# neu-vi/Superpoints_Registration

Hardware: AMD Instinct MI355X
Metric: point-cloud pairs/sec (16 384 pts/cloud) (higher is better)
Workload: dtype f32 (matrix products: range-scaled split-f16x2 MFMA, f32 accumulate; attention weights below 2^-5 of their row sum carried in one f16 plane); 1 GPU; synthetic 16384-pt pairs, full KPConv backbone + superpoint attn + Sinkhorn-SVD pose (3dmatch config, BASELINE configs[1]); streams_per_gpu=1, points_per_cloud=16384, generator=box, point_order=reference, upsample_indices=True, cross_step_overlap=True, streams_inside_a_forward=3: main path, pyramid searches, ResNet shortcut branches

## Files before the change

### superpoints_registration_amd/csrc/linear.hip

```cpp
#include <atomic>

#include "attn_planes.h"
#include "lds_dma.h"
#include "spr_common.h"
#include "split_mma.h"

namespace spr {
namespace {

constexpr int BK = 32;
static_assert(BK == kPlaneK, "the split kernels stage split_mma.h's slabs");
constexpr int LDSK = BK + 1;

template <int ACT, bool RES>
__device__ __forceinline__ float store_tile(const f32x16& acc, int row0, int col, int M, int N,
                                            float bv, const float* __restrict__ residual,
                                            float* __restrict__ out, int lh, float unscale = 1.0f,
                                            const float* __restrict__ epi = nullptr) {
  if (col >= N) return 0.f;
  float vmax = 0.f;
  float res[16];
  if (RES) {
#pragma unroll
    for (int r = 0; r < 16; ++r) {
// ... 174 lines not shown

  f32x4 ra[BM * BK / 4 / NT], rb[BN * BK / 4 / NT];
  auto load_slab = [&](int k0) {
    slab_load<BM, NT>(ra, X, M, K, tid, m0, k0);
    slab_load<BN, NT>(rb, Wt, N, K, tid, n0, k0);
  };
  auto store_slab = [&]() {
    wait_vm<0>();
    __builtin_amdgcn_sched_barrier(0);
    slab_store<BM, NT>(ra, sa, Ah, Al, tid);
    slab_store<BN, NT>(rb, sb, Bh, Bl, tid);
  };

  load_slab(0);
  for (int k0 = 0; k0 < K; k0 += BK) {
    store_slab();
    __syncthreads();
    if (k0 + BK < K) load_slab(k0 + BK);
    __builtin_amdgcn_sched_barrier(0);
#pragma unroll
    for (int s = 0; s < BK / 16; ++s) {
      const int ko = 16 * s + 8 * lh;
      f16x8 ah[TM], al[TM], bh[TN], bl[TN];
#pragma unroll
      for (int i = 0; i < TM; ++i) frag_ld40(Ah, Al, (wm * TM + i) * 32 + l31, ko, ah[i], al[i]);
#pragma unroll
      for (int j = 0; j < TN; ++j) frag_ld40(Bh, Bl, (wn * TN + j) * 32 + l31, ko, bh[j], bl[j]);
#pragma unroll
      for (int i = 0; i < TM; ++i)
#pragma unroll
        for (int j = 0; j < TN; ++j) {
          if (PLANES) acc[i][j] = mma3_32<true>(bh[j], bl[j], ah[i], al[i], acc[i][j]);
          else acc[i][j] = mma3_32(ah[i], al[i], bh[j], bl[j], acc[i][j]);
        }
    }
    __builtin_amdgcn_sched_barrier(0);
    __syncthreads();
  }
  wait_vm<0>();
  if (PLANES) {
#pragma unroll
    for (int i = 0; i < TM; ++i) {
      const int tok = m0 + (wm * TM + i) * 32 + l31;
      if (tok >= M) continue;
      const int which = (f0 + n0) >> 8;
      const float pmul = pl.scales[which];
      int vcol = 0;
      if (which == 2) {
        const int sg = find_segment(pl.cu, pl.nseg, tok);
        vcol = attn_vperm(attn_vstart_of(pl.cu[sg], sg) + tok - pl.cu[sg]);
      }
#pragma unroll
      for (int j = 0; j < TN; ++j) {
        const int fl = n0 + (wn * TN + j) * 32;
        const int fg = (f0 + fl) & 255;
        if (which == 2) {
#pragma unroll
          for (int r = 0; r < 16; r += 2) {
            const int d = acc_row32(r, lh);
            const float a = acc[i][j][r] * unscale + bias[fl + d];
            const float b = acc[i][j][r + 1] * unscale + bias[fl + d + 1];
            unsigned int hu, lu;
            split_pk_s(a, b, pmul, hu, lu);
            const f16x2 hh = __builtin_bit_cast(f16x2, hu), ll = __builtin_bit_cast(f16x2, lu);
            const size_t o = attn_v_off(fg + d, (size_t)vcol, 256);
            pl.vth[o] = hh[0];
            pl.vth[o + 16] = hh[1];
            pl.vtl[o] = ll[0];
            pl.vtl[o + 16] = ll[1];
          }
        } else {
          _Float16* ph = which == 0 ? pl.qh : pl.kh;
          _Float16* pw = which == 0 ? pl.ql : pl.kl;
          const size_t row = ((size_t)(fg >> 5) * pl.t_total + tok) * 32;
#pragma unroll
          for (int g = 0; g < 4; ++g) {
            const int d0 = 8 * g + 4 * lh;
            f32x4 v;
#pragma unroll
            for (int e = 0; e < 4; ++e) v[e] = acc[i][j][4 * g + e] * unscale + bias[fl + d0 + e];
            split_store4(v, pmul, ph + row + d0, pw + row + d0);
          }
        }
      }
    }
    return;
  }
  float omax = 0.f;
#pragma unroll
  for (int j = 0; j < TN; ++j) {
    const int col = n0 + (wn * TN + j) * 32 + l31;
    const float bv = (ACT < kEpiScale && bias && col < N) ? bias[col] : 0.f;
#pragma unroll
    for (int i = 0; i < TM; ++i)
      omax = fmaxf(omax, store_tile<ACT, RES>(acc[i][j], m0 + (wm * TM + i) * 32, col, M, N, bv, residual, out, lh,
                                              unscale, ACT >= kEpiScale ? bias : nullptr));
  }
  if (out_parts != nullptr) {
    float* shf = reinterpret_cast<float*>(gemm_smem);
    omax = wave_max(omax);
    __syncthreads();
    if (lane == 0) shf[wave] = omax;
    __syncthreads();
    if (tid == 0) {
      float t = shf[0];
      for (int w_ = 1; w_ < WM * WN; ++w_) t = fmaxf(t, shf[w_]);
      out_parts[blockIdx.x] = t;
    }
  }
}

template <int ACT>
__global__ __launch_bounds__(512) void k_gemm_nt_h3p(
    const float* __restrict__ X, int M, const float* __restrict__ Wt, int N,
    const float* __restrict__ bias, float* __restrict__ out,
    const float* __restrict__ a_parts, int n_aparts, const float* __restrict__ w_parts, int n_wparts,
    float* __restrict__ out_parts, int ntiles) {
  constexpr int K = 256, NSLAB = K / BK;
  constexpr int BM = 128, BN = 256, WN = 4, NT = 512, TM = 2, TN = 2;
  constexpr int QPS = 16 / NSLAB;
  extern __shared__ __align__(16) unsigned char gemm_smem[];
  _Float16* Ah = reinterpret_cast<_Float16*>(gemm_smem);
  _Float16* Al = Ah + BM * kPlaneStride;
  _Float16* Bh = Al + BM * kPlaneStride;
  _Float16* Bl = Bh + BN * kPlaneStride;
  const int tid = threadIdx.x, wave = tid >> 6, lane = tid & 63;
  const int wm = wave / WN, wn = wave % WN;
  const int l31 = lane & 31, lh = lane >> 5;
  const int gx = (N + BN - 1) / BN;

  float sa, sb, unscale;
  {
    float* shf = reinterpret_cast<float*>(gemm_smem);
    const int ka = pow2_exp_for(block_absmax(a_parts, shf, n_aparts));
    const int kb = pow2_exp_for(block_absmax(w_parts, shf, n_wparts));
    __syncthreads();
    sa = pow2f(ka);
    sb = pow2f(kb);
    unscale = pow2f(-ka - kb);
  }

  f32x16 acc[TM][TN], prev[TM][TN];
  f32x4 ra[BM * BK / 4 / NT], rb[BN * BK / 4 / NT];
  auto load_slab = [&](int m0, int n0, int k0) {
    slab_load<BM, NT>(ra, X, M, K, tid, m0, k0);
    slab_load<BN, NT>(rb, Wt, N, K, tid, n0, k0);
  };
  auto store_slab = [&]() {
    slab_store<BM, NT>(ra, sa, Ah, Al, tid);
    slab_store<BN, NT>(rb, sb, Bh, Bl, tid);
  };

  bool have_prev = false;
  int pm0 = 0, pn0 = 0, ptile = 0;
  float pbias[TN] = {0.f, 0.f};
  float pmax = 0.f;
  auto emit = [&](auto qtag) {
    constexpr int Q = decltype(qtag)::value;
    constexpr int b = Q >> 2, g = Q & 3, bi = b >> 1, bj = b & 1;
    const int row0 = pm0 + (wm * TM + bi) * 32 + 8 * g + 4 * lh;
    const int col = pn0 + (wn * TN + bj) * 32 + l31;
    if (col < N) {
      float* p = out + (size_t)row0 * N + col;
#pragma unroll
      for (int e = 0; e < 4; ++e) {
        float y = prev[bi][bj][4 * g + e] * unscale + pbias[bj];
        if (ACT == SPR_ACT_RELU) y = fmaxf(y, 0.f);
        if (ACT == SPR_ACT_SIGMOID) y = 1.f / (1.f + expf(-y));
        if (row0 + e < M) {
          asm volatile("global_store_dword %0, %1, off" ::"v"(p + (size_t)e * N), "v"(y) : "memory");
          pmax = fmaxf(pmax, fabsf(y));
        }
      }
    }
  };
  auto publish_prev_max = [&]() {
    if (out_parts == nullptr) return;
    float* shf = reinterpret_cast<float*>(gemm_smem);
    const float t_ = wave_max(pmax);
    __syncthreads();
    if (lane == 0) shf[wave] = t_;
    __syncthreads();
    if (tid == 0) {
      float m_ = shf[0];
      for (int w_ = 1; w_ < 8; ++w_) m_ = fmaxf(m_, shf[w_]);
      out_parts[ptile] = m_;
    }
    __syncthreads();
    pmax = 0.f;
  };

  int t = blockIdx.x;
  if (t < ntiles) {
    const int lid = xcd_swizzle(t, ntiles);
    load_slab((lid / gx) * BM, (lid % gx) * BN, 0);
  }
  bool young = false;
  for (; t < ntiles; t += gridDim.x) {
    const int lid = xcd_swizzle(t, ntiles);
    const int m0 = (lid / gx) * BM, n0 = (lid % gx) * BN;
    const int tn = t + gridDim.x;
    int nm0 = 0, nn0 = 0;
    if (tn < ntiles) {
      const int nl = xcd_swizzle(tn, ntiles);
      nm0 = (nl / gx) * BM;
      nn0 = (nl % gx) * BN;
    }
#pragma unroll
    for (int i = 0; i < TM; ++i)
#pragma unroll
      for (int j = 0; j < TN; ++j)
#pragma unroll
        for (int r = 0; r < 16; ++r) acc[i][j][r] = 0.f;
    auto slab = [&](auto stag) {
      constexpr int S = decltype(stag)::value;
      if (young) wait_vm<8>();
      else wait_vm<0>();
      __builtin_amdgcn_sched_barrier(0);
      store_slab();
      __syncthreads();
      if (S + 1 < NSLAB) load_slab(m0, n0, (S + 1) * BK);
      else if (tn < ntiles) load_slab(nm0, nn0, 0);
      __builtin_amdgcn_sched_barrier(0);
#pragma unroll
      for (int ks = 0; ks < BK / 16; ++ks) {
        const int ko = 16 * ks + 8 * lh;
        f16x8 ah[TM], al[TM], bh[TN], bl[TN];
#pragma unroll
        for (int i = 0; i < TM; ++i) frag_ld40(Ah, Al, (wm * TM + i) * 32 + l31, ko, ah[i], al[i]);
#pragma unroll
        for (int j = 0; j < TN; ++j) frag_ld40(Bh, Bl, (wn * TN + j) * 32 + l31, ko, bh[j], bl[j]);
#pragma unroll
        for (int i = 0; i < TM; ++i)
#pragma unroll
          for (int j = 0; j < TN; ++j) acc[i][j] = mma3_32(ah[i], al[i], bh[j], bl[j], acc[i][j]);
      }
      __builtin_amdgcn_sched_barrier(0);
      young = false;
      if (have_prev) {
        emit(std::integral_constant<int, QPS * S>{});
        emit(std::integral_constant<int, QPS * S + 1>{});
        young = true;
      }
      __builtin_amdgcn_sched_barrier(0);
      __syncthreads();
    };
    slab(std::integral_constant<int, 0>{});
    slab(std::integral_constant<int, 1>{});
    slab(std::integral_constant<int, 2>{});
    slab(std::integral_constant<int, 3>{});
    slab(std::integral_constant<int, 4>{});
    slab(std::integral_constant<int, 5>{});
    slab(std::integral_constant<int, 6>{});
    slab(std::integral_constant<int, 7>{});
    if (have_prev) publish_prev_max();
#pragma unroll
    for (int i = 0; i < TM; ++i)
#pragma unroll
      for (int j = 0; j < TN; ++j) prev[i][j] = acc[i][j];
    pm0 = m0;
    pn0 = n0;
    ptile = t;
#pragma unroll
    for (int j = 0; j < TN; ++j) {
      const int col = n0 + (wn * TN + j) * 32 + l31;
      pbias[j] = (bias && col < N) ? bias[col] : 0.f;
    }
    have_prev = true;
  }
  if (have_prev) {
    emit(std::integral_constant<int, 0>{});  emit(std::integral_constant<int, 1>{});
    emit(std::integral_constant<int, 2>{});  emit(std::integral_constant<int, 3>{});
    emit(std::integral_constant<int, 4>{});  emit(std::integral_constant<int, 5>{});
    emit(std::integral_constant<int, 6>{});  emit(std::integral_constant<int, 7>{});
    emit(std::integral_constant<int, 8>{});  emit(std::integral_constant<int, 9>{});
    emit(std::integral_constant<int, 10>{}); emit(std::integral_constant<int, 11>{});
    emit(std::integral_constant<int, 12>{}); emit(std::integral_constant<int, 13>{});
    emit(std::integral_constant<int, 14>{}); emit(std::integral_constant<int, 15>{});
    publish_prev_max();
  }
}

static std::atomic<int> g_gemm_mode{1};

__global__ void k_gemv_rows(const float* __restrict__ X, int M, int K, const float* __restrict__ Wt,
                            int N, const float* __restrict__ bias,
                            const float* __restrict__ residual, int act, float* __restrict__ out) {
  const long wid = ((long)blockIdx.x * blockDim.x + threadIdx.x) >> 6;
  const int lane = threadIdx.x & 63;
  if (wid >= (long)M * N) return;
  const int row = (int)(wid / N), n = (int)(wid % N);
  float s = 0.f;
  for (int k = lane; k < K; k += 64) s += X[(size_t)row * K + k] * Wt[(size_t)n * K + k];
  s = wave_sum(s);
  if (lane == 0) {
    float v = s + (bias ? bias[n] : 0.f);
    if (residual) v += residual[(size_t)row * N + n];
    if (act == SPR_ACT_RELU) v = fmaxf(v, 0.f);
    if (act == SPR_ACT_SIGMOID) v = 1.f / (1.f + expf(-v));
    out[(size_t)row * N + n] = v;
  }
}

constexpr int kLnRangeSlots = kRangeSlots;
template <int MAXV>
__global__ void k_layernorm(const float* __restrict__ x, int m, int c,
                            const float* __restrict__ gamma, const float* __restrict__ beta,
                            float eps, const float* __restrict__ pos, float* __restrict__ out_norm,
                            float* __restrict__ out_pos, float* __restrict__ range_norm,
                            float* __restrict__ range_pos) {
  __shared__ float shr[8];
  const int row = (blockIdx.x * blockDim.x + threadIdx.x) >> 6;
  const int lane = threadIdx.x & 63;
  float mxn = 0.f, mxp = 0.f;
  if (row < m) {
  const int nv = c >> 6;
  float v[MAXV];
  float s = 0.f;
#pragma unroll
  for (int i = 0; i < MAXV; ++i) {
    v[i] = (i < nv) ? x[(size_t)row * c + i * 64 + lane] : 0.f;
    s += v[i];
  }
  const float mean0 = wave_sum(s) / (float)c;
  float sd = 0.f;
#pragma unroll
  for (int i = 0; i < MAXV; ++i) sd += (i < nv) ? v[i] - mean0 : 0.f;
  const float mean = mean0 + wave_sum(sd) / (float)c;
  float ss = 0.f;
#pragma unroll
  for (int i = 0; i < MAXV; ++i) {
    const float d = (i < nv) ? v[i] - mean : 0.f;
    ss += d * d;
  }
  const float rstd = 1.0f / sqrtf(wave_sum(ss) / (float)c + eps);
#pragma unroll
  for (int i = 0; i < MAXV; ++i) {
    if (i < nv) {
      const int ch = i * 64 + lane;
      const float y = (v[i] - mean) * rstd * gamma[ch] + beta[ch];
      mxn = fmaxf(mxn, fabsf(y));
      if (out_norm) out_norm[(size_t)row * c + ch] = y;
      if (out_pos) {
        const float yp = y + pos[(size_t)row * c + ch];
        mxp = fmaxf(mxp, fabsf(yp));
        out_pos[(size_t)row * c + ch] = yp;
      }
    }
  }
  }
  if (range_norm || range_pos) {
    mxn = wave_max(mxn);
    mxp = wave_max(mxp);
    if (lane == 0) {
      shr[threadIdx.x >> 6] = mxn;
      shr[4 + (threadIdx.x >> 6)] = mxp;
    }
    __syncthreads();
    if (threadIdx.x == 0) {
      const int slot = blockIdx.x & (kLnRangeSlots - 1);
      if (range_norm)
        atomicMax(reinterpret_cast<unsigned int*>(range_norm) + slot,
                  __float_as_uint(fmaxf(fmaxf(shr[0], shr[1]), fmaxf(shr[2], shr[3]))));
      if (range_pos)
        atomicMax(reinterpret_cast<unsigned int*>(range_pos) + slot,
                  __float_as_uint(fmaxf(fmaxf(shr[4], shr[5]), fmaxf(shr[6], shr[7]))));
    }
  }
}

constexpr int kLnRows = 4;
__global__ __launch_bounds__(256) void k_layernorm256(const float* __restrict__ x, int m,
                                                      const float* __restrict__ gamma,
                                                      const float* __restrict__ beta, float eps,
                                                      const float* __restrict__ pos, float* __restrict__ out_norm,
                                                      float* __restrict__ out_pos, float* __restrict__ range_norm,
                                                      float* __restrict__ range_pos) {
  __shared__ float shr[8];
  const int row0 = ((blockIdx.x * blockDim.x + threadIdx.x) >> 6) * kLnRows;
  const int lane = threadIdx.x & 63;
  float mxn = 0.f, mxp = 0.f;
  float4 v[kLnRows], pv[kLnRows];
#pragma unroll
  for (int r = 0; r < kLnRows; ++r) {
    if (row0 + r < m) {
      const size_t o = (size_t)(row0 + r) * 256 + 4 * lane;
      v[r] = *reinterpret_cast<const float4*>(x + o);
      if (out_pos) pv[r] = *reinterpret_cast<const float4*>(pos + o);
    }
  }
  const float4 g = *reinterpret_cast<const float4*>(gamma + 4 * lane);
  const float4 b = *reinterpret_cast<const float4*>(beta + 4 * lane);
#pragma unroll
  for (int r = 0; r < kLnRows; ++r) {
    if (row0 + r >= m) continue;
    const size_t o = (size_t)(row0 + r) * 256 + 4 * lane;
    const float mean0 = wave_sum((v[r].x + v[r].y) + (v[r].z + v[r].w)) / 256.0f;
    const float mean = mean0 + wave_sum(((v[r].x - mean0) + (v[r].y - mean0)) + ((v[r].z - mean0) + (v[r].w - mean0))) / 256.0f;
    const float dx = v[r].x - mean, dy = v[r].y - mean, dz = v[r].z - mean, dw = v[r].w - mean;
    const float rstd = 1.0f / sqrtf(wave_sum((dx * dx + dy * dy) + (dz * dz + dw * dw)) / 256.0f + eps);
    float4 y;
    y.x = dx * rstd * g.x + b.x;
    y.y = dy * rstd * g.y + b.y;
    y.z = dz * rstd * g.z + b.z;
    y.w = dw * rstd * g.w + b.w;
    mxn = fmaxf(mxn, fmaxf(fmaxf(fabsf(y.x), fabsf(y.y)), fmaxf(fabsf(y.z), fabsf(y.w))));
    if (out_norm) *reinterpret_cast<float4*>(out_norm + o) = y;
    if (out_pos) {
      float4 yp;
      yp.x = y.x + pv[r].x;
      yp.y = y.y + pv[r].y;
      yp.z = y.z + pv[r].z;
      yp.w = y.w + pv[r].w;
      mxp = fmaxf(mxp, fmaxf(fmaxf(fabsf(yp.x), fabsf(yp.y)), fmaxf(fabsf(yp.z), fabsf(yp.w))));
      *reinterpret_cast<float4*>(out_pos + o) = yp;
    }
  }
  if (range_norm || range_pos) {
    mxn = wave_max(mxn);
    mxp = wave_max(mxp);
    if (lane == 0) {
      shr[threadIdx.x >> 6] = mxn;
      shr[4 + (threadIdx.x >> 6)] = mxp;
    }
    __syncthreads();
    if (threadIdx.x == 0) {
      const int slot = blockIdx.x & (kLnRangeSlots - 1);
      if (range_norm)
        atomicMax(reinterpret_cast<unsigned int*>(range_norm) + slot,
                  __float_as_uint(fmaxf(fmaxf(shr[0], shr[1]), fmaxf(shr[2], shr[3]))));
      if (range_pos)
        atomicMax(reinterpret_cast<unsigned int*>(range_pos) + slot,
                  __float_as_uint(fmaxf(fmaxf(shr[4], shr[5]), fmaxf(shr[6], shr[7]))));
    }
  }
}

__global__ void k_posemb(const float* __restrict__ xyz, int n, int d_model, int npf, float scale,
                         float temperature, float* __restrict__ out) {
  const long gid = (long)blockIdx.x * blockDim.x + threadIdx.x;
  if (gid >= (long)n * d_model) return;
  const int row = (int)(gid / d_model), ch = (int)(gid % d_model);
  float v = 0.f;
  if (ch < 3 * npf) {
    const int axis = ch / npf, i = ch % npf;
    const float e = (float)(2 * (i / 2)) / (float)npf;
    const float dim_t = powf(temperature, e);
    const float a = (xyz[3 * (size_t)row + axis] * scale) / dim_t;
    v = (i & 1) ? cosf(a) : sinf(a);
  }
  out[gid] = v;
}

}
}

using namespace spr;

namespace {
template <int ACT, bool RES>
int launch_gemm(const float* x, int m, int k, const float* w, int n, const float* bias,
                const float* residual, float* out, const float* a_parts, int n_aparts, const float* w_parts,
                int n_wparts, float* out_parts, int out_cap, int* out_n, hipStream_t stream) {
  if (out_n) *out_n = 0;
  if (spr::g_gemm_mode.load(std::memory_order_relaxed) == 1) {
    SPR_REQUIRE(a_parts != nullptr && w_parts != nullptr, "linear: split-fp16 mode needs the absmax partials");
    auto lds = [](int bm, int bn) { return (size_t)(bm + bn) * spr::kPlaneStride * 2 * sizeof(_Float16); };
    if (!RES && ACT <= SPR_ACT_SIGMOID && n >= 256 && k == 256 && m >= 1024 && m < 32768) {
      auto kern = spr::k_gemm_nt_h3p<ACT>;
      if (int rc = ensure_dyn_lds((const void*)kern, (int)lds(128, 256))) return rc;
      const int ntiles = cdiv(n, 256) * cdiv(m, 128);
      int grid = device_cu_count();
      grid = grid < ntiles ? grid : ntiles;
      if (grid >= 8) grid &= ~7;
      float* op = (out_parts && ntiles <= out_cap) ? out_parts : nullptr;
      if (op && out_n) *out_n = ntiles;
      hipLaunchKernelGGL(kern, dim3(grid), dim3(512), lds(128, 256), stream, x, m, w, n, bias, out,
                         a_parts, n_aparts, w_parts, n_wparts, op, ntiles);
    } else if (n >= 256 && m >= 256 && cdiv(n, 256) * cdiv(m, 256) >= 128) {
      auto kern = spr::k_gemm_nt_h3<256, 256, 4, 2, ACT, RES>;
      if (int rc = ensure_dyn_lds((const void*)kern, (int)lds(256, 256))) return rc;
      const int grid = cdiv(n, 256) * cdiv(m, 256);
      float* op = (out_parts && grid <= out_cap) ? out_parts : nullptr;
      if (op && out_n) *out_n = grid;
      hipLaunchKernelGGL(kern, dim3(grid), dim3(512), lds(256, 256), stream, x, m, k,
                         w, n, bias, residual, out, spr::AttnPlanes(), 0, a_parts, n_aparts, w_parts, op, (const spr::GemmGroup*)nullptr, n_wparts);
    } else if (n > 32) {
      const int grid = cdiv(n, 64) * cdiv(m, 128);
      float* op = (out_parts && grid <= out_cap) ? out_parts : nullptr;
      if (op && out_n) *out_n = grid;
      hipLaunchKernelGGL((spr::k_gemm_nt_h3<128, 64, 4, 1, ACT, RES>), dim3(grid),
                         dim3(256), lds(128, 64), stream, x, m, k, w, n, bias, residual, out, spr::AttnPlanes(), 0,
                         a_parts, n_aparts, w_parts, op, (const spr::GemmGroup*)nullptr, n_wparts);
    } else {
      hipLaunchKernelGGL((spr::k_gemm_nt_h3<128, 32, 4, 1, ACT, RES>), dim3(cdiv(n, 32) * cdiv(m, 128)),
                         dim3(256), lds(128, 32), stream, x, m, k, w, n, bias, residual, out, spr::AttnPlanes(), 0,
                         a_parts, n_aparts, w_parts, (float*)nullptr, (const spr::GemmGroup*)nullptr, n_wparts);
    }
  } else if (n % 64 == 0) {
    hipLaunchKernelGGL((spr::k_gemm_nt<2, 2, ACT, RES>), dim3((n / 64) * cdiv(m, 64)), dim3(256), 0, stream,
                       x, m, k, w, n, bias, residual, out);
  } else {
    hipLaunchKernelGGL((spr::k_gemm_nt<4, 1, ACT, RES>), dim3(cdiv(n, 32) * cdiv(m, 128)), dim3(256), 0,
                       stream, x, m, k, w, n, bias, residual, out);
  }
  SPR_LAUNCH_CHECK();
  return 0;
}
}

int spr::gemm_mode() { return spr::g_gemm_mode.load(std::memory_order_relaxed); }

int spr::launch_inproj_planes(const float* x, int m, int k, const float* w, int n, const float* bias, int f0,
                              const AttnPlanes& planes, const float* a_parts, int n_aparts, const float* w_parts,
                              hipStream_t stream) {
  SPR_REQUIRE(n % 256 == 0 && f0 % 256 == 0 && k % BK == 0 && m >= 1 && bias != nullptr,
              "in-projection planes: bad shape (m=%d k=%d n=%d)", m, k, n);
  SPR_REQUIRE(a_parts && w_parts && planes.scales, "in-projection planes: missing scale inputs");
  auto kern = spr::k_gemm_nt_h3<256, 256, 4, 2, SPR_ACT_NONE, false, true>;
  const size_t lds = (size_t)(256 + 256) * spr::kPlaneStride * 2 * sizeof(_Float16);
  if (int rc = ensure_dyn_lds((const void*)kern, (int)lds)) return rc;
  hipLaunchKernelGGL(kern, dim3(cdiv(n, 256) * cdiv(m, 256)), dim3(512), lds, stream, x, m, k, w, n, bias,
                     (const float*)nullptr, (float*)nullptr, planes, f0, a_parts, n_aparts, w_parts, (float*)nullptr,
                     (const spr::GemmGroup*)nullptr, kAmaxParts);
  SPR_LAUNCH_CHECK();
  return 0;
}

int spr::launch_linear_ranged(const float* x, int m, int k, const float* w, int n, const float* bias,
                              float* out, const float* a_parts, const float* w_parts, hipStream_t stream) {
  return launch_gemm<SPR_ACT_NONE, false>(x, m, k, w, n, bias, nullptr, out, a_parts, kAmaxParts, w_parts, kAmaxParts,
                                          nullptr, 0, nullptr, stream);
}

void spr::gemm_group_tile(int max_n, int* bm, int* bn) {
  if (max_n >= 256) { *bm = 256; *bn = 256; }
  else if (max_n > 32) { *bm = 128; *bn = 64; }
  else { *bm = 128; *bn = 32; }
}

namespace {
template <int ACT>
int launch_grouped_act(const float* a, int k, const float* b, float* c, const spr::GemmGroup* groups_dev,
                       int total_tiles, int max_n, const float* a_parts, const float* w_parts, const float* epi,
                       hipStream_t stream) {
  auto lds = [](int bm, int bn) { return (size_t)(bm + bn) * spr::kPlaneStride * 2 * sizeof(_Float16); };
  int bm, bn;
  spr::gemm_group_tile(max_n, &bm, &bn);
  if (bn == 256) {
    auto kern = spr::k_gemm_nt_h3<256, 256, 4, 2, ACT, false>;
    if (int rc = ensure_dyn_lds((const void*)kern, (int)lds(256, 256))) return rc;
    hipLaunchKernelGGL(kern, dim3(total_tiles), dim3(512), lds(256, 256), stream, a, 0, k, b, 0, epi,
                       (const float*)nullptr, c, spr::AttnPlanes(), 0, a_parts, kAmaxParts, w_parts,
                       (float*)nullptr, groups_dev, kAmaxParts);
  } else if (bn == 64) {
    hipLaunchKernelGGL((spr::k_gemm_nt_h3<128, 64, 4, 1, ACT, false>), dim3(total_tiles), dim3(256),
                       lds(128, 64), stream, a, 0, k, b, 0, epi, (const float*)nullptr, c, spr::AttnPlanes(), 0,
                       a_parts, kAmaxParts, w_parts, (float*)nullptr, groups_dev, kAmaxParts);
  } else {
    hipLaunchKernelGGL((spr::k_gemm_nt_h3<128, 32, 4, 1, ACT, false>), dim3(total_tiles), dim3(256),
                       lds(128, 32), stream, a, 0, k, b, 0, epi, (const float*)nullptr, c, spr::AttnPlanes(), 0,
                       a_parts, kAmaxParts, w_parts, (float*)nullptr, groups_dev, kAmaxParts);
  }
  SPR_LAUNCH_CHECK();
  return 0;
}
}

int spr::launch_gemm_grouped(const float* a, int k, const float* b, float* c, const GemmGroup* groups_dev,
                             int total_tiles, int max_n, const float* a_parts, const float* w_parts,
                             int epi_mode, const float* epi, hipStream_t stream) {
  SPR_REQUIRE(spr::gemm_mode() == 1 && a_parts && w_parts && groups_dev && total_tiles >= 1 && k % BK == 0,
              "grouped gemm: bad arguments");
  SPR_REQUIRE(epi_mode == 0 || epi != nullptr, "grouped gemm: epilogue parameters missing");
  switch (epi_mode) {
    case 0: return launch_grouped_act<SPR_ACT_NONE>(a, k, b, c, groups_dev, total_tiles, max_n, a_parts, w_parts,
                                                    nullptr, stream);
    case kEpiScale: return launch_grouped_act<kEpiScale>(a, k, b, c, groups_dev, total_tiles, max_n, a_parts,
                                                         w_parts, epi, stream);
  }
  SPR_REQUIRE(false, "grouped gemm: unknown epilogue %d", epi_mode);
  return 1;
}

namespace {
struct LinearWs {
  float *ap, *wp;
};
LinearWs linear_layout(Workspace& w) {
  LinearWs l;
  l.ap = w.take<float>(kAmaxParts);
  l.wp = w.take<float>(kAmaxParts);
  return l;
}
}

extern "C" size_t spr_linear_workspace_bytes(void) {
  return measure(linear_layout);
}

extern "C" int spr_linear(const float* x, int m, int k, const float* w, int n, const float* bias,
                          const float* residual, int act, float* out, const float* x_range, int x_range_n,
                          const float* w_range, int w_range_n, float* out_range, int out_range_cap,
                          int* out_range_n_host, void* ws, size_t ws_bytes, void* stream_) {
  hipStream_t stream = (hipStream_t)stream_;
  if (out_range_n_host) *out_range_n_host = 0;
  SPR_REQUIRE(m > 0 && k > 0 && n > 0, "linear: bad sizes m=%d k=%d n=%d", m, k, n);
  SPR_REQUIRE(act >= 0 && act <= 2, "linear: unknown activation %d", act);
  SPR_REQUIRE(x_range == nullptr || x_range_n >= 1, "linear: x_range needs a count");
  SPR_REQUIRE(w_range == nullptr || w_range_n >= 1, "linear: w_range needs a count");
  if (n < 16 || k % BK != 0) {
    SPR_REQUIRE(n <= 64 || k % BK == 0, "linear: k must be a multiple of %d for n > 64 (k=%d n=%d)", BK, k, n);
    const long waves = (long)m * n;
    hipLaunchKernelGGL(k_gemv_rows, dim3(cdiv(waves * 64, 256)), dim3(256), 0, stream, x, m, k, w, n,
                       bias, residual, act, out);
    SPR_LAUNCH_CHECK();
    return 0;
  }
  const float *a_parts = nullptr, *w_parts = nullptr;
  int n_ap = kAmaxParts, n_wp = kAmaxParts;
  if (spr::gemm_mode() == 1) {
    Workspace wk(ws, ws_bytes);
    const auto [ap, wp] = linear_layout(wk);
    SPR_REQUIRE(ws != nullptr && wk.ok(),
                "linear: workspace too small (%zu bytes given, spr_linear_workspace_bytes() needed)", ws_bytes);
    a_parts = x_range != nullptr ? x_range : ap;
    w_parts = w_range != nullptr ? w_range : wp;
    if (x_range != nullptr) n_ap = x_range_n;
    if (w_range != nullptr) n_wp = w_range_n;
    if (x_range == nullptr && w_range == nullptr) {
      if (int rc = launch_absmax2(x, m, k, k, ap, w, n, k, k, wp, stream)) return rc;
    } else if (x_range == nullptr) {
      if (int rc = launch_absmax(x, m, k, k, ap, stream)) return rc;
    } else if (w_range == nullptr) {
      if (int rc = launch_absmax(w, n, k, k, wp, stream)) return rc;
    }
  }
  const bool res = residual != nullptr;
#define SPR_LG(A, R) launch_gemm<A, R>(x, m, k, w, n, bias, residual, out, a_parts, n_ap, w_parts, n_wp, out_range, \
                                       out_range_cap, out_range_n_host, stream)
  switch (act * 2 + (res ? 1 : 0)) {
    case 0: return SPR_LG(SPR_ACT_NONE, false);
    case 1: return SPR_LG(SPR_ACT_NONE, true);
    case 2: return SPR_LG(SPR_ACT_RELU, false);
    case 3: return SPR_LG(SPR_ACT_RELU, true);
    case 4: return SPR_LG(SPR_ACT_SIGMOID, false);
    default: return SPR_LG(SPR_ACT_SIGMOID, true);
  }
#undef SPR_LG
}

extern "C" int spr_set_gemm_mode(int mode) {
  SPR_REQUIRE(mode == 0 || mode == 1, "gemm mode must be 0 (exact f32 MFMA) or 1 (split-fp16)");
  spr::g_gemm_mode.store(mode);
  return 0;
}

extern "C" int spr_layernorm_range_count(int m) {
  (void)m;
  return kLnRangeSlots;
}

extern "C" int spr_layernorm(const float* x, int m, int c, const float* gamma, const float* beta,
                             float eps, const float* pos, float* out_norm, float* out_pos, float* range_norm,
                             float* range_pos, void* stream_) {
  hipStream_t stream = (hipStream_t)stream_;
  SPR_REQUIRE(m > 0 && c % 64 == 0 && c <= 1024, "layernorm: c must be a multiple of 64 and <= 1024 (c=%d)", c);
  SPR_REQUIRE(out_pos == nullptr || pos != nullptr, "layernorm: out_pos needs pos");
  const int grid = cdiv((long)m * 64, 256);
  if (c == 256)
    hipLaunchKernelGGL(k_layernorm256, dim3(cdiv((long)cdiv(m, kLnRows) * 64, 256)), dim3(256), 0, stream, x, m, gamma, beta, eps, pos, out_norm,
                       out_pos, range_norm, range_pos);
  else if (c <= 256)
    hipLaunchKernelGGL(k_layernorm<4>, dim3(grid), dim3(256), 0, stream, x, m, c, gamma, beta, eps,
                       pos, out_norm, out_pos, range_norm, range_pos);
  else
    hipLaunchKernelGGL(k_layernorm<16>, dim3(grid), dim3(256), 0, stream, x, m, c, gamma, beta, eps,
                       pos, out_norm, out_pos, range_norm, range_pos);
  SPR_LAUNCH_CHECK();
  return 0;
}

extern "C" int spr_posemb_sine(const float* xyz, int n, int d_model, float scale, float temperature,
                               float* out, void* stream_) {
  hipStream_t stream = (hipStream_t)stream_;
  SPR_REQUIRE(n > 0 && d_model >= 6, "posemb: bad sizes");
  const int npf = d_model / 3 / 2 * 2;
  const long total = (long)n * d_model;
  hipLaunchKernelGGL(k_posemb, dim3(cdiv(total, 256)), dim3(256), 0, stream, xyz, n, d_model, npf,
                     scale, temperature, out);
  SPR_LAUNCH_CHECK();
  return 0;
}
```

### superpoints_registration_amd/csrc/norm_pool.hip

```cpp
#include "spr_common.h"

namespace spr {
namespace {

constexpr int kSliceRows = 512;
int in_nsplit(int max_len) {
  int s = cdiv(max_len > 0 ? max_len : 1, kSliceRows);
  return s < 1 ? 1 : s;
}

__global__ __launch_bounds__(256) void k_in_stats(const float* __restrict__ x,
                                                  const int* __restrict__ cu, int c, int nsplit,
                                                  double* __restrict__ part ) {
  const int cloud = blockIdx.x, split = blockIdx.y, cb = blockIdx.z * 64;
  const int beg = cu[cloud], end = cu[cloud + 1];
  const int r0 = beg + split * kSliceRows;
  const int r1 = min(r0 + kSliceRows, end);
  const int cw = min(c - cb, 64);
  const int cw4 = cw >> 2;
  const int rl = 256 / cw4;
  const int tc = threadIdx.x % cw4, tr = threadIdx.x / cw4;
  __shared__ double sh[8][256];
  double s[4] = {0, 0, 0, 0}, ss[4] = {0, 0, 0, 0};
  if (tr < rl) {
    const float* base = x + cb + 4 * tc;
    int r = r0 + tr;
    for (; r + 3 * rl < r1; r += 4 * rl) {
      float4 v[4];
#pragma unroll
      for (int u = 0; u < 4; ++u)
        v[u] = *reinterpret_cast<const float4*>(base + (size_t)(r + u * rl) * c);
#pragma unroll
      for (int u = 0; u < 4; ++u) {
        const double a = v[u].x, b = v[u].y, cc = v[u].z, d = v[u].w;
        s[0] += a; ss[0] += a * a;
        s[1] += b; ss[1] += b * b;
        s[2] += cc; ss[2] += cc * cc;
        s[3] += d; ss[3] += d * d;
      }
    }
    for (; r < r1; r += rl) {
      const float4 v = *reinterpret_cast<const float4*>(base + (size_t)r * c);
      const double a = v.x, b = v.y, cc = v.z, d = v.w;
      s[0] += a; ss[0] += a * a;
      s[1] += b; ss[1] += b * b;
      s[2] += cc; ss[2] += cc * cc;
      s[3] += d; ss[3] += d * d;
    }
  }
#pragma unroll
  for (int k = 0; k < 4; ++k) {
    sh[k][threadIdx.x] = s[k];
    sh[4 + k][threadIdx.x] = ss[k];
  }
  __syncthreads();
  if (tr == 0) {
    double* p = part + (((size_t)cloud * nsplit + split) * 2) * c;
#pragma unroll
    for (int k = 0; k < 4; ++k) {
      double a = s[k], b = ss[k];
      for (int q = 1; q < rl; ++q) {
        a += sh[k][q * cw4 + tc];
        b += sh[4 + k][q * cw4 + tc];
      }
      p[cb + 4 * tc + k] = a;
      p[c + cb + 4 * tc + k] = b;
    }
  }
}

__global__ void k_in_final(const double* __restrict__ part, const int* __restrict__ cu, int nb,
                           int c, int nsplit, float eps, float* __restrict__ mean,
                           float* __restrict__ rstd) {
  const int i = blockIdx.x * blockDim.x + threadIdx.x;
  if (i >= nb * c) return;
  const int cloud = i / c, ch = i % c;
  double s = 0.0, ss = 0.0;
  for (int k = 0; k < nsplit; ++k) {
    const double* p = part + (((size_t)cloud * nsplit + k) * 2) * c;
    s += p[ch];
    ss += p[c + ch];
  }
  const int len = cu[cloud + 1] - cu[cloud];
  const double n = len > 0 ? (double)len : 1.0;
  const double m = s / n;
  double var = ss / n - m * m;
  if (var < 0.0) var = 0.0;
  mean[i] = (float)m;
  rstd[i] = (float)(1.0 / sqrt(var + (double)eps));
}

__device__ __forceinline__ void publish_range(float mx, float* __restrict__ slots, int nslots) {
  __shared__ float shr[4];
  mx = wave_max(mx);
  if ((threadIdx.x & 63) == 0) shr[threadIdx.x >> 6] = mx;
  __syncthreads();
  if (threadIdx.x == 0)
    atomicMax(reinterpret_cast<unsigned int*>(slots) + (blockIdx.x & (nslots - 1)),
              __float_as_uint(fmaxf(fmaxf(shr[0], shr[1]), fmaxf(shr[2], shr[3]))));
}

constexpr int kInApplyUnroll = 4;
__global__ __launch_bounds__(256) void k_in_apply(const float* __restrict__ x, const int* __restrict__ cu, int n,
                                                  int nb, int c, int norm, const float* __restrict__ mean,
                                                  const float* __restrict__ rstd, const float* __restrict__ add,
                                                  float slope, float* __restrict__ out,
                                                  float* __restrict__ out_range, int nslots) {
  const int c4 = c >> 2;
  const long total = (long)n * c4;
  const long stride = (long)gridDim.x * blockDim.x;
  const long g0 = (long)blockIdx.x * blockDim.x + threadIdx.x;
  float4 v[kInApplyUnroll], a[kInApplyUnroll];
#pragma unroll
  for (int u = 0; u < kInApplyUnroll; ++u) {
    const long gid = g0 + u * stride;
    if (gid < total) {
      v[u] = reinterpret_cast<const float4*>(x)[gid];
      if (add) a[u] = reinterpret_cast<const float4*>(add)[gid];
    }
  }
  float mx = 0.f;
#pragma unroll
  for (int u = 0; u < kInApplyUnroll; ++u) {
    const long gid = g0 + u * stride;
    if (gid >= total) continue;
    float4 w = v[u];
    if (norm) {
      const int row = (int)(gid / c4), q = (int)(gid % c4);
      const int cloud = find_segment(cu, nb, row);
      const float4 m = reinterpret_cast<const float4*>(mean + (size_t)cloud * c)[q];
      const float4 r = reinterpret_cast<const float4*>(rstd + (size_t)cloud * c)[q];
      w.x = (w.x - m.x) * r.x;
      w.y = (w.y - m.y) * r.y;
      w.z = (w.z - m.z) * r.z;
      w.w = (w.w - m.w) * r.w;
    }
    if (add) {
      w.x += a[u].x;
      w.y += a[u].y;
      w.z += a[u].z;
      w.w += a[u].w;
    }
    w.x = w.x >= 0.f ? w.x : w.x * slope;
    w.y = w.y >= 0.f ? w.y : w.y * slope;
    w.z = w.z >= 0.f ? w.z : w.z * slope;
    w.w = w.w >= 0.f ? w.w : w.w * slope;
    reinterpret_cast<float4*>(out)[gid] = w;
    mx = fmaxf(mx, fmaxf(fmaxf(fabsf(w.x), fabsf(w.y)), fmaxf(fabsf(w.z), fabsf(w.w))));
  }
  if (out_range != nullptr) publish_range(mx, out_range, nslots);
}

__global__ __launch_bounds__(256) void k_in_bwd_stats(const float* __restrict__ x, const float* __restrict__ out,
                                                      const float* __restrict__ dout, const int* __restrict__ cu,
                                                      int c, int nsplit, float slope,
                                                      const float* __restrict__ mean, const float* __restrict__ rstd,
                                                      double* __restrict__ part ) {
  const int cloud = blockIdx.x, split = blockIdx.y, cb = blockIdx.z * 64;
  const int beg = cu[cloud], end = cu[cloud + 1];
  const int r0 = beg + split * kSliceRows;
  const int r1 = min(r0 + kSliceRows, end);
  const int cw = min(c - cb, 64);
  const int cw4 = cw >> 2;
  const int rl = 256 / cw4;
  const int tc = threadIdx.x % cw4, tr = threadIdx.x / cw4;
  __shared__ double sh[8][256];
  double s1[4] = {0, 0, 0, 0}, s2[4] = {0, 0, 0, 0};
  if (tr < rl) {
    const int col = cb + 4 * tc;
    const float4 mu = *reinterpret_cast<const float4*>(mean + (size_t)cloud * c + col);
    const float4 rs = *reinterpret_cast<const float4*>(rstd + (size_t)cloud * c + col);
    for (int r = r0 + tr; r < r1; r += rl) {
      const size_t o = (size_t)r * c + col;
      const float4 xv = *reinterpret_cast<const float4*>(x + o);
      const float4 ov = *reinterpret_cast<const float4*>(out + o);
      const float4 dv = *reinterpret_cast<const float4*>(dout + o);
      const float g0 = dv.x * (ov.x > 0.f ? 1.f : slope), g1 = dv.y * (ov.y > 0.f ? 1.f : slope);
      const float g2 = dv.z * (ov.z > 0.f ? 1.f : slope), g3 = dv.w * (ov.w > 0.f ? 1.f : slope);
      s1[0] += (double)g0; s2[0] += (double)g0 * (double)((xv.x - mu.x) * rs.x);
      s1[1] += (double)g1; s2[1] += (double)g1 * (double)((xv.y - mu.y) * rs.y);
      s1[2] += (double)g2; s2[2] += (double)g2 * (double)((xv.z - mu.z) * rs.z);
      s1[3] += (double)g3; s2[3] += (double)g3 * (double)((xv.w - mu.w) * rs.w);
    }
  }
#pragma unroll
  for (int k = 0; k < 4; ++k) {
    sh[k][threadIdx.x] = s1[k];
    sh[4 + k][threadIdx.x] = s2[k];
  }
  __syncthreads();
  if (tr == 0) {
    double* p = part + (((size_t)cloud * nsplit + split) * 2) * c;
#pragma unroll
    for (int k = 0; k < 4; ++k) {
      double a = s1[k], b = s2[k];
      for (int q = 1; q < rl; ++q) {
        a += sh[k][q * cw4 + tc];
        b += sh[4 + k][q * cw4 + tc];
      }
      p[cb + 4 * tc + k] = a;
      p[c + cb + 4 * tc + k] = b;
    }
  }
}

__global__ void k_in_bwd_final(const double* __restrict__ part, const int* __restrict__ cu, int nb, int c,
                               int nsplit, double* __restrict__ m1, double* __restrict__ m2) {
  const int i = blockIdx.x * blockDim.x + threadIdx.x;
  if (i >= nb * c) return;
  const int cloud = i / c, ch = i % c;
  double s1 = 0.0, s2 = 0.0;
  for (int k = 0; k < nsplit; ++k) {
    const double* p = part + (((size_t)cloud * nsplit + k) * 2) * c;
    s1 += p[ch];
    s2 += p[c + ch];
  }
  const int len = cu[cloud + 1] - cu[cloud];
  const double n = len > 0 ? (double)len : 1.0;
  m1[i] = s1 / n;
  m2[i] = s2 / n;
}

__global__ void k_in_bwd_apply(const float* __restrict__ x, const float* __restrict__ out,
                               const float* __restrict__ dout, const int* __restrict__ cu, int n, int nb, int c,
                               int norm, float slope, const float* __restrict__ mean,
                               const float* __restrict__ rstd, const double* __restrict__ m1,
                               const double* __restrict__ m2, float* __restrict__ dx, float* __restrict__ dadd) {
  const long gid = (long)blockIdx.x * blockDim.x + threadIdx.x;
  if (gid >= (long)n * c) return;
  const int row = (int)(gid / c), ch = (int)(gid % c);
  const float g = dout[gid] * (out[gid] > 0.f ? 1.f : slope);
  if (dadd) dadd[gid] = g;
  if (!norm) {
    dx[gid] = g;
    return;
  }
  const int cloud = find_segment(cu, nb, row);
  const size_t s = (size_t)cloud * c + ch;
  const float xh = (x[gid] - mean[s]) * rstd[s];
  dx[gid] = rstd[s] * (float)(((double)g - m1[s]) - (double)xh * m2[s]);
}

__global__ void k_in_bwd_apply4(const float* __restrict__ x, const float* __restrict__ out,
                                const float* __restrict__ dout, const int* __restrict__ cu, int n, int nb, int c,
                                int norm, float slope, const float* __restrict__ mean,
                                const float* __restrict__ rstd, const double* __restrict__ m1,
                                const double* __restrict__ m2, float* __restrict__ dx, float* __restrict__ dadd) {
  const int c4 = c >> 2;
  const long gid = (long)blockIdx.x * blockDim.x + threadIdx.x;
  if (gid >= (long)n * c4) return;
  const int row = (int)(gid / c4), ch = 4 * (int)(gid % c4);
  const float4 d4 = reinterpret_cast<const float4*>(dout)[gid], o4 = reinterpret_cast<const float4*>(out)[gid];
  float g[4] = {d4.x * (o4.x > 0.f ? 1.f : slope), d4.y * (o4.y > 0.f ? 1.f : slope),
                d4.z * (o4.z > 0.f ? 1.f : slope), d4.w * (o4.w > 0.f ? 1.f : slope)};
  if (dadd) reinterpret_cast<float4*>(dadd)[gid] = make_float4(g[0], g[1], g[2], g[3]);
  if (!norm) {
    reinterpret_cast<float4*>(dx)[gid] = make_float4(g[0], g[1], g[2], g[3]);
    return;
  }
  const int cloud = find_segment(cu, nb, row);
  const size_t s = (size_t)cloud * c + ch;
  const float4 x4 = reinterpret_cast<const float4*>(x)[gid];
  const float xv[4] = {x4.x, x4.y, x4.z, x4.w};
  float r[4];
#pragma unroll
  for (int e = 0; e < 4; ++e) {
    const float xh = (xv[e] - mean[s + e]) * rstd[s + e];
    r[e] = rstd[s + e] * (float)(((double)g[e] - m1[s + e]) - (double)xh * m2[s + e]);
  }
  reinterpret_cast<float4*>(dx)[gid] = make_float4(r[0], r[1], r[2], r[3]);
}

__global__ void k_maxpool(const float* __restrict__ x, int ns, int c, const int* __restrict__ idx,
                          int nq, int idx_stride, int k, float* __restrict__ out, float* __restrict__ out_range,
                          int nslots, const int* __restrict__ order) {
  const int c4 = c >> 2;
  long gid = (long)blockIdx.x * blockDim.x + threadIdx.x;
  if (order != nullptr) gid = ((long)(blockIdx.x & 7) * (gridDim.x >> 3) + (blockIdx.x >> 3)) * blockDim.x + threadIdx.x;
  float mx = 0.f;
  if (gid < (long)nq * c4) {
  const int q = (int)(gid % c4);
  const int row = order != nullptr ? order[gid / c4] : (int)(gid / c4);
  gid = (long)row * c4 + q;
  float4 m = make_float4(-INFINITY, -INFINITY, -INFINITY, -INFINITY);
  const int* ir = idx + (size_t)row * idx_stride;
  int j = 0;
  for (; j + 4 <= k; j += 4) {
    int id[4];
    float4 v[4];
#pragma unroll
    for (int u = 0; u < 4; ++u) id[u] = ir[j + u];
#pragma unroll
    for (int u = 0; u < 4; ++u) {
      v[u] = make_float4(0.f, 0.f, 0.f, 0.f);
      if (id[u] >= 0 && id[u] < ns) v[u] = reinterpret_cast<const float4*>(x + (size_t)id[u] * c)[q];
    }
#pragma unroll
    for (int u = 0; u < 4; ++u) {
      m.x = fmaxf(m.x, v[u].x);
      m.y = fmaxf(m.y, v[u].y);
      m.z = fmaxf(m.z, v[u].z);
      m.w = fmaxf(m.w, v[u].w);
    }
  }
  for (; j < k; ++j) {
    const int id = ir[j];
    float4 v = make_float4(0.f, 0.f, 0.f, 0.f);
    if (id >= 0 && id < ns) v = reinterpret_cast<const float4*>(x + (size_t)id * c)[q];
    m.x = fmaxf(m.x, v.x);
    m.y = fmaxf(m.y, v.y);
    m.z = fmaxf(m.z, v.z);
    m.w = fmaxf(m.w, v.w);
  }
  reinterpret_cast<float4*>(out)[gid] = m;
  mx = fmaxf(fmaxf(fabsf(m.x), fabsf(m.y)), fmaxf(fabsf(m.z), fabsf(m.w)));
  }
  if (out_range != nullptr) publish_range(mx, out_range, nslots);
}

__global__ void k_gather_rows(const float* __restrict__ x, int n_src, int c,
                              const int* __restrict__ idx, int n, float* __restrict__ out) {
  const long gid = (long)blockIdx.x * blockDim.x + threadIdx.x;
  if (gid >= (long)n * c) return;
  const int row = (int)(gid / c), ch = (int)(gid % c);
  const int id = idx[row];
  out[gid] = (id >= 0 && id < n_src) ? x[(size_t)id * c + ch] : 0.f;
}

}
}

using namespace spr;

namespace {
struct InstnormWs {
  double* part;
  float *mean, *rstd;
  double *m1, *m2;
};
InstnormWs instnorm_layout(Workspace& w, int max_len, int nb, int c, bool backward) {
  const size_t B = (size_t)(nb > 0 ? nb : 1), C = (size_t)(c > 0 ? c : 1);
  InstnormWs l{};
  l.part = w.take<double>(B * in_nsplit(max_len) * 2 * C);
  l.mean = w.take<float>(B * C);
  l.rstd = w.take<float>(B * C);
  if (backward) {
    l.m1 = w.take<double>(B * C);
    l.m2 = w.take<double>(B * C);
  }
  return l;
}
}

extern "C" size_t spr_instnorm_workspace_bytes(int max_len, int nb, int c) {
  return measure(instnorm_layout, max_len, nb, c, false);
}

extern "C" int spr_instnorm(const float* x, const int* cu, int n, int nb, int max_len_host, int c,
                            float eps, int norm, const float* add, float slope, float* out, float* out_range,
                            int out_range_n, void* ws, size_t ws_bytes, void* stream_) {
  hipStream_t stream = (hipStream_t)stream_;
  SPR_REQUIRE(out_range == nullptr || (out_range_n >= 1 && (out_range_n & (out_range_n - 1)) == 0),
              "instnorm: out_range_n must be a power of two");
  SPR_REQUIRE(n > 0 && nb >= 1 && c >= 4 && c % 4 == 0, "instnorm: need n>0 and c %% 4 == 0 (c=%d)", c);
  float* mean = nullptr;
  float* rstd = nullptr;
  if (norm) {
    SPR_REQUIRE(max_len_host >= 1 && max_len_host <= n, "instnorm: bad max_len_host=%d", max_len_host);
    Workspace w(ws, ws_bytes);
    const InstnormWs l = instnorm_layout(w, max_len_host, nb, c, false);
    SPR_REQUIRE(ws != nullptr && w.ok(), "instnorm: workspace too small");
    const int nsplit = in_nsplit(max_len_host);
    double* part = l.part;
    mean = l.mean;
    rstd = l.rstd;
    hipLaunchKernelGGL(k_in_stats, dim3(nb, nsplit, cdiv(c, 64)), dim3(256), 0, stream, x, cu, c, nsplit, part);
    hipLaunchKernelGGL(k_in_final, dim3(cdiv((long)nb * c, 256)), dim3(256), 0, stream, part, cu,
                       nb, c, nsplit, eps, mean, rstd);
    SPR_LAUNCH_CHECK();
  }
  const long total = (long)n * (c / 4);
  hipLaunchKernelGGL(k_in_apply, dim3(cdiv(total, 256 * kInApplyUnroll)), dim3(256), 0, stream, x, cu, n, nb, c,
                     norm, mean, rstd, add, slope, out, out_range, out_range_n);
  SPR_LAUNCH_CHECK();
  return 0;
}

extern "C" int spr_instnorm_stats(const float* x, const int* cu, int n, int nb, int max_len_host, int c, float eps,
                                  float* mean, float* rstd, void* ws, size_t ws_bytes, void* stream_) {
  hipStream_t stream = (hipStream_t)stream_;
  SPR_REQUIRE(x && cu && mean && rstd && n > 0 && nb >= 1 && c >= 4 && c % 4 == 0, "instnorm_stats: bad arguments (c=%d)", c);
  SPR_REQUIRE(max_len_host >= 1 && max_len_host <= n, "instnorm_stats: bad max_len_host=%d", max_len_host);
  Workspace w(ws, ws_bytes);
  double* part = instnorm_layout(w, max_len_host, nb, c, false).part;
  SPR_REQUIRE(ws != nullptr && w.ok(), "instnorm_stats: workspace too small");
  const int nsplit = in_nsplit(max_len_host);
  hipLaunchKernelGGL(k_in_stats, dim3(nb, nsplit, cdiv(c, 64)), dim3(256), 0, stream, x, cu, c, nsplit, part);
  hipLaunchKernelGGL(k_in_final, dim3(cdiv((long)nb * c, 256)), dim3(256), 0, stream, part, cu, nb, c, nsplit, eps, mean,
                     rstd);
  SPR_LAUNCH_CHECK();
  return 0;
}

extern "C" size_t spr_instnorm_bwd_workspace_bytes(int max_len, int nb, int c) {
  return measure(instnorm_layout, max_len, nb, c, true);
}

extern "C" int spr_instnorm_bwd(const float* x, const float* out, const float* dout, const int* cu, int n, int nb,
                                int max_len_host, int c, float eps, int norm, float slope, float* dx, float* dadd,
                                void* ws, size_t ws_bytes, void* stream_) {
  hipStream_t stream = (hipStream_t)stream_;
  SPR_REQUIRE(n > 0 && nb >= 1 && c >= 4 && c % 4 == 0, "instnorm_bwd: need n>0 and c %% 4 == 0 (c=%d)", c);
  SPR_REQUIRE(x && out && dout && dx, "instnorm_bwd: null operand");
  float *mean = nullptr, *rstd = nullptr;
  double *m1 = nullptr, *m2 = nullptr;
  if (norm) {
    SPR_REQUIRE(max_len_host >= 1 && max_len_host <= n, "instnorm_bwd: bad max_len_host=%d", max_len_host);
    Workspace w(ws, ws_bytes);
    const InstnormWs l = instnorm_layout(w, max_len_host, nb, c, true);
    SPR_REQUIRE(ws != nullptr && w.ok(), "instnorm_bwd: workspace too small");
    const int nsplit = in_nsplit(max_len_host);
    double* part = l.part;
    mean = l.mean; rstd = l.rstd; m1 = l.m1; m2 = l.m2;
    hipLaunchKernelGGL(k_in_stats, dim3(nb, nsplit, cdiv(c, 64)), dim3(256), 0, stream, x, cu, c, nsplit, part);
    hipLaunchKernelGGL(k_in_final, dim3(cdiv((long)nb * c, 256)), dim3(256), 0, stream, part, cu, nb, c, nsplit,
                       eps, mean, rstd);
    hipLaunchKernelGGL(k_in_bwd_stats, dim3(nb, nsplit, cdiv(c, 64)), dim3(256), 0, stream, x, out, dout, cu, c, nsplit, slope,
                       mean, rstd, part);
    hipLaunchKernelGGL(k_in_bwd_final, dim3(cdiv((long)nb * c, 256)), dim3(256), 0, stream, part, cu, nb, c, nsplit,
                       m1, m2);
    SPR_LAUNCH_CHECK();
  }
  if (c % 4 == 0 && (((uintptr_t)x | (uintptr_t)out | (uintptr_t)dout | (uintptr_t)dx | (uintptr_t)dadd) & 15) == 0)
    hipLaunchKernelGGL(k_in_bwd_apply4, dim3(cdiv((long)n * (c / 4), 256)), dim3(256), 0, stream, x, out, dout, cu, n, nb,
                       c, norm, slope, mean, rstd, m1, m2, dx, dadd);
  else
    hipLaunchKernelGGL(k_in_bwd_apply, dim3(cdiv((long)n * c, 256)), dim3(256), 0, stream, x, out, dout, cu, n, nb, c,
                       norm, slope, mean, rstd, m1, m2, dx, dadd);
  SPR_LAUNCH_CHECK();
  return 0;
}

extern "C" int spr_maxpool_gather(const float* x, int ns, int c, const int* idx, int nq, int idx_stride, int k,
                                  const int* order, float* out, float* out_range, int out_range_n, void* stream_) {
  hipStream_t stream = (hipStream_t)stream_;
  SPR_REQUIRE(out_range == nullptr || (out_range_n >= 1 && (out_range_n & (out_range_n - 1)) == 0),
              "maxpool: out_range_n must be a power of two");
  SPR_REQUIRE(nq > 0 && ns > 0 && c % 4 == 0 && k >= 1 && k <= idx_stride, "maxpool: bad arguments");
  const long total = (long)nq * (c / 4);
  const long nblk = order != nullptr ? align_up((size_t)cdiv(total, 256), 8) : cdiv(total, 256);
  hipLaunchKernelGGL(k_maxpool, dim3((unsigned)nblk), dim3(256), 0, stream, x, ns, c, idx, nq, idx_stride, k, out,
                     out_range, out_range_n, order);
  SPR_LAUNCH_CHECK();
  return 0;
}

extern "C" int spr_gather_rows(const float* x, int n_src, int c, const int* idx, int n, float* out,
                               void* stream_) {
  hipStream_t stream = (hipStream_t)stream_;
  SPR_REQUIRE(n > 0 && c >= 1, "gather_rows: bad arguments");
  const long total = (long)n * c;
  hipLaunchKernelGGL(k_gather_rows, dim3(cdiv(total, 256)), dim3(256), 0, stream, x, n_src, c, idx,
                     n, out);
  SPR_LAUNCH_CHECK();
  return 0;
}
```

Baseline: 1269 pairs/s.

## Add specialized kernels for n=1 GEMV, paired posemb, and live-neighbor maxpool

Adds a GEMV kernel for single-output linears that processes four rows per wave and reuses the weight vector across them. Adds a positional-embedding kernel that precomputes the frequency table in shared memory and writes sin/cos pairs as float2. Adds a maxpool kernel that compacts valid neighbor indices with ballots and issues batched buffer loads, skipping invalid neighbors. The three changes are unrelated and each targets a small kernel, so the end-to-end effect depends on how much time these kernels take within the full pipeline.

```diff
diff --git a/superpoints_registration_amd/csrc/linear.hip b/superpoints_registration_amd/csrc/linear.hip
--- a/superpoints_registration_amd/csrc/linear.hip
+++ b/superpoints_registration_amd/csrc/linear.hip
@@ -500,6 +500,46 @@
   }
 }
 
+constexpr int kGemvRows = 4;
+__global__ __launch_bounds__(256) void k_gemv_rows_n1(const float* __restrict__ X, int M, int K,
+                                                      const float* __restrict__ Wt, const float* __restrict__ bias,
+                                                      const float* __restrict__ residual, int act,
+                                                      float* __restrict__ out) {
+  const long row0 = (((long)blockIdx.x * blockDim.x + threadIdx.x) >> 6) * kGemvRows;
+  const int lane = threadIdx.x & 63;
+  if (row0 >= M) return;
+  float s[kGemvRows];
+#pragma unroll
+  for (int r = 0; r < kGemvRows; ++r) s[r] = 0.f;
+  for (int k0 = 0; k0 < K; k0 += 256) {
+    float xv[kGemvRows][4], wv[4];
+#pragma unroll
+    for (int r = 0; r < kGemvRows; ++r) {
+      const long row = row0 + r < M ? row0 + r : M - 1;
+#pragma unroll
+      for (int i = 0; i < 4; ++i) xv[r][i] = X[(size_t)row * K + k0 + 64 * i + lane];
+    }
+#pragma unroll
+    for (int i = 0; i < 4; ++i) wv[i] = Wt[k0 + 64 * i + lane];
+#pragma unroll
+    for (int r = 0; r < kGemvRows; ++r)
+#pragma unroll
+      for (int i = 0; i < 4; ++i) s[r] += xv[r][i] * wv[i];
+  }
+#pragma unroll
+  for (int r = 0; r < kGemvRows; ++r) {
+    const float t = wave_sum(s[r]);
+    const long row = row0 + r;
+    if (lane == 0 && row < M) {
+      float v = t + (bias ? bias[0] : 0.f);
+      if (residual) v += residual[row];
+      if (act == SPR_ACT_RELU) v = fmaxf(v, 0.f);
+      if (act == SPR_ACT_SIGMOID) v = 1.f / (1.f + expf(-v));
+      out[row] = v;
+    }
+  }
+}
+
 constexpr int kLnRangeSlots = kRangeSlots;
 template <int MAXV>
 __global__ void k_layernorm(const float* __restrict__ x, int m, int c,
@@ -648,6 +688,29 @@
     v = (i & 1) ? cosf(a) : sinf(a);
   }
   out[gid] = v;
+}
+
+constexpr int kPosembMaxPairs = 1024;
+constexpr int kPosembSteps = 4;
+__global__ __launch_bounds__(256) void k_posemb_pairs(const float* __restrict__ xyz, int n, int d_model, int npf,
+                                                      float scale, float temperature, float* __restrict__ out) {
+  __shared__ float dim_t[kPosembMaxPairs];
+  const int hp = npf >> 1, slots = d_model >> 1;
+  for (int i = threadIdx.x; i < hp; i += 256) dim_t[i] = powf(temperature, (float)(2 * i) / (float)npf);
+  __syncthreads();
+#pragma unroll
+  for (int u = 0; u < kPosembSteps; ++u) {
+    const long gid = ((long)blockIdx.x * kPosembSteps + u) * 256 + threadIdx.x;
+    if (gid >= (long)n * slots) return;
+    const int row = (int)(gid / slots), s = (int)(gid % slots);
+    float2 v = make_float2(0.f, 0.f);
+    if (s < 3 * hp) {
+      const int axis = s / hp, i = s % hp;
+      const float a = (xyz[3 * (size_t)row + axis] * scale) / dim_t[i];
+      v = make_float2(sinf(a), cosf(a));
+    }
+    reinterpret_cast<float2*>(out)[gid] = v;
+  }
 }
 
 }
@@ -810,8 +873,12 @@
   if (n < 16 || k % BK != 0) {
     SPR_REQUIRE(n <= 64 || k % BK == 0, "linear: k must be a multiple of %d for n > 64 (k=%d n=%d)", BK, k, n);
     const long waves = (long)m * n;
-    hipLaunchKernelGGL(k_gemv_rows, dim3(cdiv(waves * 64, 256)), dim3(256), 0, stream, x, m, k, w, n,
-                       bias, residual, act, out);
+    if (n == 1 && k % 256 == 0)
+      hipLaunchKernelGGL(k_gemv_rows_n1, dim3(cdiv((long)cdiv(m, kGemvRows) * 64, 256)), dim3(256), 0, stream, x, m, k,
+                         w, bias, residual, act, out);
+    else
+      hipLaunchKernelGGL(k_gemv_rows, dim3(cdiv(waves * 64, 256)), dim3(256), 0, stream, x, m, k, w, n,
+                         bias, residual, act, out);
     SPR_LAUNCH_CHECK();
     return 0;
   }
@@ -885,8 +952,12 @@
   SPR_REQUIRE(n > 0 && d_model >= 6, "posemb: bad sizes");
   const int npf = d_model / 3 / 2 * 2;
   const long total = (long)n * d_model;
-  hipLaunchKernelGGL(k_posemb, dim3(cdiv(total, 256)), dim3(256), 0, stream, xyz, n, d_model, npf,
-                     scale, temperature, out);
+  if (d_model % 2 == 0 && npf / 2 <= kPosembMaxPairs && ((uintptr_t)out & 7) == 0)
+    hipLaunchKernelGGL(k_posemb_pairs, dim3(cdiv(total / 2, 256 * kPosembSteps)), dim3(256), 0, stream, xyz, n, d_model, npf, scale,
+                       temperature, out);
+  else
+    hipLaunchKernelGGL(k_posemb, dim3(cdiv(total, 256)), dim3(256), 0, stream, xyz, n, d_model, npf,
+                       scale, temperature, out);
   SPR_LAUNCH_CHECK();
   return 0;
 }
diff --git a/superpoints_registration_amd/csrc/norm_pool.hip b/superpoints_registration_amd/csrc/norm_pool.hip
--- a/superpoints_registration_amd/csrc/norm_pool.hip
+++ b/superpoints_registration_amd/csrc/norm_pool.hip
@@ -318,6 +318,88 @@
   if (out_range != nullptr) publish_range(mx, out_range, nslots);
 }
 
+constexpr int kMpFlight = 8;
+constexpr unsigned kMpOff = 0x80000000u;
+template <int G>
+__global__ __launch_bounds__(256) void k_maxpool_live(const float* __restrict__ x, int ns, const int* __restrict__ idx,
+                                                      int nq, int idx_stride, int k, float* __restrict__ out,
+                                                      float* __restrict__ out_range, int nslots,
+                                                      const int* __restrict__ order) {
+  constexpr int c = 4 * G, QW = 64 / G;
+  using Mask = std::conditional_t<G == 64, unsigned long long, unsigned int>;
+  const int lane = threadIdx.x & 63, gl = lane & (G - 1), gb = lane - gl;
+  long vb = blockIdx.x;
+  if (order != nullptr) vb = (long)(blockIdx.x & 7) * (gridDim.x >> 3) + (blockIdx.x >> 3);
+  const long p = vb * (4 * QW) + (threadIdx.x >> 6) * QW + (lane / G);
+  const bool valid = p < nq;
+  int row = 0;
+  if (valid) row = order != nullptr ? order[p] : (int)p;
+  const int* ir = idx + (size_t)row * idx_stride;
+  const auto xr = __builtin_amdgcn_make_buffer_rsrc(const_cast<float*>(x), 0, (int)((size_t)ns * c * sizeof(float)),
+                                                    0x00020000);
+  float4 m = make_float4(-INFINITY, -INFINITY, -INFINITY, -INFINITY);
+  bool dead = false;
+  int id = (valid && gl < k) ? ir[gl] : -1;
+  for (int base = 0; base < k; base += G) {
+    const int col = base + gl;
+    int idn = -1;
+    if (valid && col + G < k) idn = ir[col + G];
+    const bool in = valid && col < k;
+    const bool live = in && id >= 0 && id < ns;
+    const unsigned long long lm = __ballot(live), dm = __ballot(in && !live);
+    Mask gm;
+    if constexpr (G == 64) {
+      gm = lm;
+      dead |= dm != 0;
+    } else {
+      constexpr Mask kGroup = (Mask)(~0ull >> (64 - G));
+      gm = (Mask)(lm >> gb) & kGroup;
+      dead |= ((Mask)(dm >> gb) & kGroup) != 0;
+    }
+    bool more;
+    if constexpr (G == 64) more = gm != 0; else more = __any(gm != 0);
+    while (more) {
+      unsigned off[kMpFlight];
+      bool have[kMpFlight];
+#pragma unroll
+      for (int u = 0; u < kMpFlight; ++u) {
+        have[u] = gm != 0;
+        const int b = have[u] ? (int)__builtin_ctzll((unsigned long long)gm) : 0;
+        gm &= gm - 1;
+        int idu;
+        if constexpr (G == 64) idu = __builtin_amdgcn_readlane(id, b);
+        else idu = __shfl(id, gb + b, 64);
+        off[u] = have[u] ? (unsigned)idu * (unsigned)(c * sizeof(float)) + 16u * gl : kMpOff;
+      }
+      decltype(__builtin_amdgcn_raw_buffer_load_b128(xr, 0, 0, 0)) raw[kMpFlight];
+#pragma unroll
+      for (int u = 0; u < kMpFlight; ++u) raw[u] = __builtin_amdgcn_raw_buffer_load_b128(xr, off[u], 0, 0);
+      __builtin_amdgcn_sched_barrier(0);
+#pragma unroll
+      for (int u = 0; u < kMpFlight; ++u) {
+        m.x = fmaxf(m.x, have[u] ? __uint_as_float(raw[u][0]) : -INFINITY);
+        m.y = fmaxf(m.y, have[u] ? __uint_as_float(raw[u][1]) : -INFINITY);
+        m.z = fmaxf(m.z, have[u] ? __uint_as_float(raw[u][2]) : -INFINITY);
+        m.w = fmaxf(m.w, have[u] ? __uint_as_float(raw[u][3]) : -INFINITY);
+      }
+      if constexpr (G == 64) more = gm != 0; else more = __any(gm != 0);
+    }
+    id = idn;
+  }
+  float mx = 0.f;
+  if (valid) {
+    if (dead) {
+      m.x = fmaxf(m.x, 0.f);
+      m.y = fmaxf(m.y, 0.f);
+      m.z = fmaxf(m.z, 0.f);
+      m.w = fmaxf(m.w, 0.f);
+    }
+    *reinterpret_cast<float4*>(out + (size_t)row * c + 4 * gl) = m;
+    mx = fmaxf(fmaxf(fabsf(m.x), fabsf(m.y)), fmaxf(fabsf(m.z), fabsf(m.w)));
+  }
+  if (out_range != nullptr) publish_range(mx, out_range, nslots);
+}
+
 __global__ void k_gather_rows(const float* __restrict__ x, int n_src, int c,
                               const int* __restrict__ idx, int n, float* __restrict__ out) {
   const long gid = (long)blockIdx.x * blockDim.x + threadIdx.x;
@@ -449,8 +531,17 @@
   SPR_REQUIRE(nq > 0 && ns > 0 && c % 4 == 0 && k >= 1 && k <= idx_stride, "maxpool: bad arguments");
   const long total = (long)nq * (c / 4);
   const long nblk = order != nullptr ? align_up((size_t)cdiv(total, 256), 8) : cdiv(total, 256);
-  hipLaunchKernelGGL(k_maxpool, dim3((unsigned)nblk), dim3(256), 0, stream, x, ns, c, idx, nq, idx_stride, k, out,
-                     out_range, out_range_n, order);
+#define SPR_MP_LIVE(G)                                                                                               \
+  hipLaunchKernelGGL(k_maxpool_live<G>, dim3((unsigned)nblk), dim3(256), 0, stream, x, ns, idx, nq, idx_stride, k, \
+                     out, out_range, out_range_n, order)
+  const bool fits = (size_t)ns * c * sizeof(float) < kMpOff;
+  if (c == 256 && fits) SPR_MP_LIVE(64);
+  else if (c == 128 && fits) SPR_MP_LIVE(32);
+  else if (c == 64 && fits) SPR_MP_LIVE(16);
+  else
+    hipLaunchKernelGGL(k_maxpool, dim3((unsigned)nblk), dim3(256), 0, stream, x, ns, c, idx, nq, idx_stride, k, out,
+                       out_range, out_range_n, order);
+#undef SPR_MP_LIVE
   SPR_LAUNCH_CHECK();
   return 0;
 }
```

Result: no change. 1276 pairs/s (median of 6 runs) (+0.5%).
